# tonyzyl/ladcast

Hardware: AMD Instinct MI355X
Metric: ensemble-member-steps/sec (higher is better)
Workload: dtype f32

## Files before the change

include/ladcast_hip.h:

```cpp
#ifndef LADCAST_HIP_H
#define LADCAST_HIP_H

#ifdef __cplusplus
extern "C" {
#endif

#define LDC_ABI_VERSION 5

#define LDC_OK 0
#define LDC_ERR_ARG (-1)
#define LDC_ERR_ALIGN (-2)
#define LDC_ERR_UNSUPPORTED (-3)

enum ldc_act { LDC_ACT_NONE = 0, LDC_ACT_SILU = 1, LDC_ACT_GELU_TANH = 2, LDC_ACT_RELU = 3 };
#define LDC_ACT_IN_TIMESTEP_SINCOS 16

int ldc_abi_version(void);
const char* ldc_build_arch(void);

typedef struct ldc_gemm_desc {
  int M, N, K, batch;
  int lda, ldw, ldc, ldr;
  long long a_bs, c_bs, r_bs;
  int gate_bs;
  int act;
  int flags;
  int reserved;
} ldc_gemm_desc;
#define LDC_GEMM_A_SPLIT 1
#define LDC_GEMM_C_SPLIT 2
#define LDC_GEMM_BF16_1TERM 4
#define LDC_GEMM_F32_REGSTAGE 8
#define LDC_FMT_F32 0
#define LDC_FMT_SPLIT 1
#define LDC_FMT_BF16 2
int ldc_sizeof_gemm_desc(void);
int ldc_gemm_bias_act(const float* A, const float* W, const float* bias, const float* gate,
                      const float* R, float* C, const ldc_gemm_desc* d, void* stream);

#define LDC_GEMM_MAX_PROBLEMS 4
typedef struct ldc_gemm_problem {
  const float* A;
  const float* W;
  const float* bias;
  const float* gate;
  const float* R;
  float* C;
  ldc_gemm_desc d;
} ldc_gemm_problem;
int ldc_sizeof_gemm_problem(void);
long long ldc_gemm_grouped_workspace_bytes(void);
int ldc_gemm_grouped_workspace_init(void* workspace, long long workspace_bytes, void* stream);
int ldc_gemm_grouped(const ldc_gemm_problem* problems, int n, void* workspace, long long workspace_bytes,
// ... 66 lines not shown
int ldc_attn_fwd_split_qrows(const float* Q, const float* K, const float* V, float* O, int B, int S, int Sq, int H, int ld_qkv,
                             long long qkv_bs, int ldo, long long o_bs, const float* key_bias, int flags, void* workspace,
                             long long workspace_bytes, void* stream);

int ldc_qk_rmsnorm_rope(float* q, float* k, int B, int row0, int rows, int H, int ld, long long bs,
                        const float* wq, const float* wk, float eps, const float* cos_tab,
                        const float* sin_tab, void* stream);

int ldc_layernorm_mod(const float* x, float* y, int B, int rows, int D, int ldx, long long x_bs,
                      int ldy, long long y_bs, const float* scale, const float* shift, int mod_bs,
                      int mode, float eps, int out_split, void* stream);
int ldc_layernorm_mod2(const float* x, float* y, int B, int rows, int D, int ldx, long long x_bs,
                       int ldy, long long y_bs, const float* scale, const float* shift, int split_row,
                       const float* scale2, const float* shift2, int mod_bs, int mode, float eps,
                       int out_split, void* stream);

int ldc_mean_rows(const float* x, float* y, int B, int rows, int D, int ldx, long long x_bs, void* stream);
int ldc_mean_rows_split(const float* x, float* y, float* x_split, int B, int rows, int D, int ldx,
                        long long x_bs, int lds, long long s_bs, int fmt , void* stream);

int ldc_gate_residual(const float* resid, const float* y, const float* gate, float* out, int B,
                      int rows, int D, int ld_res, long long res_bs, int ld_y, long long y_bs,
                      int gate_bs, void* stream);
int ldc_gate_residual_layernorm(float* resid, const float* y, const float* gate, float* out, int B, int rows, int D, int ld_res,
                                long long res_bs, int ld_y, long long y_bs, int gate_bs, int ld_out, long long out_bs,
                                const float* weight, const float* bias, float eps, int out_split, void* stream);

int ldc_chan_to_token(const float* in, float* out, int B, int C, int N, int ldo, int fill_cols, void* stream);
int ldc_chan_to_token_split(const float* in, float* out, int B, int C, int N, int ldo, int fill_cols,
                            int out_split, void* stream);
// ... 202 lines not shown
```

ladcast_amd/csrc/gemm_f32.hip:

```cpp
#include "common.h"

namespace {

constexpr int BM = 128, BN = 128, BK = 32;
constexpr int LDP = 36;
constexpr int STAGE_FLOATS = (BM + BN) * LDP;

struct GemmArgs {
  const float* A;
  const float* W;
  const float* bias;
  const float* gate;
  const float* R;
  float* C;
  ldc_gemm_desc d;
  int cH, cW, cin, ks;
};

__device__ __forceinline__ int sphere_src_pixel(int h, int w, int ky, int kx, int H, int W, int ks) {
  const int p = ks >> 1;
  if ((h == 0 && ky < p) || (h == H - 1 && ky >= ks - p)) kx = ks - 1 - kx;
  int r = h + ky - p;
  int c = w + kx - p;
  if (r < 0) {
    r = -1 - r;
    c -= W >> 1;
  } else if (r >= H) {
    r = 2 * H - 1 - r;
    c -= W >> 1;
  }
  c %= W;
// ... 67 lines not shown
        rb[i] = (kin && gn < N) ? *reinterpret_cast<const float4*>(W + static_cast<long long>(gn) * ldw + kk)
                                : make_float4(0.f, 0.f, 0.f, 0.f);
      }
    }
  };
  auto sstore = [&](int stage) {
    float* As = smem + stage * STAGE_FLOATS;
    float* Bs = As + BM * LDP;
#pragma unroll
    for (int i = 0; i < 4; ++i) {
      const int row = r0 + 32 * i;
      *reinterpret_cast<float4*>(As + row * LDP + c4 * 4) = ra[i];
      *reinterpret_cast<float4*>(Bs + row * LDP + c4 * 4) = rb[i];
    }
  };

  f32x16 acc[2][2];
#pragma unroll
  for (int i = 0; i < 2; ++i)
#pragma unroll
    for (int j = 0; j < 2; ++j)
#pragma unroll
      for (int r = 0; r < 16; ++r) acc[i][j][r] = 0.f;

  const int nk = CONV ? ktpt * p.ks * p.ks : (K + BK - 1) / BK;
  gload(0);
  sstore(0);
  __syncthreads();

  const int frag_row = lane & 31;
  const int frag_k = (lane >> 5) * 4;

  for (int kt = 0; kt < nk; ++kt) {
    if (kt + 1 < nk) gload(kt + 1);
    const float* As = smem + (kt & 1) * STAGE_FLOATS;
    const float* Bs = As + BM * LDP;
    const float* a_base = As + (wm * 64 + frag_row) * LDP + frag_k;
    const float* b_base = Bs + (wn * 64 + frag_row) * LDP + frag_k;
#pragma unroll
    for (int kg = 0; kg < 4; ++kg) {
      const float4 a0 = *reinterpret_cast<const float4*>(a_base + kg * 8);
      const float4 a1 = *reinterpret_cast<const float4*>(a_base + 32 * LDP + kg * 8);
      const float4 b0 = *reinterpret_cast<const float4*>(b_base + kg * 8);
      const float4 b1 = *reinterpret_cast<const float4*>(b_base + 32 * LDP + kg * 8);
      const float av[2][4] = {{a0.x, a0.y, a0.z, a0.w}, {a1.x, a1.y, a1.z, a1.w}};
      const float bv[2][4] = {{b0.x, b0.y, b0.z, b0.w}, {b1.x, b1.y, b1.z, b1.w}};
#pragma unroll
      for (int r = 0; r < 4; ++r)
#pragma unroll
        for (int i = 0; i < 2; ++i)
#pragma unroll
          for (int j = 0; j < 2; ++j)
            acc[i][j] = __builtin_amdgcn_mfma_f32_32x32x2f32(av[i][r], bv[j][r], acc[i][j], 0, 0, 0);
    }
    if (kt + 1 < nk) sstore((kt + 1) & 1);
    __syncthreads();
  }

  float* __restrict__ C = p.C + static_cast<long long>(b) * p.d.c_bs;
  const float* __restrict__ R = p.R ? p.R + static_cast<long long>(b) * p.d.r_bs : nullptr;
  const float* __restrict__ gate = p.gate ? p.gate + static_cast<long long>(b) * p.d.gate_bs : nullptr;
  const int act = p.d.act;
#pragma unroll
  for (int j = 0; j < 2; ++j) {
    const int n = bn * BN + wn * 64 + j * 32 + (lane & 31);
    if (n >= N) continue;
    const float bias_n = p.bias ? p.bias[n] : 0.f;
    const float gate_n = gate ? gate[n] : 1.f;
#pragma unroll
    for (int i = 0; i < 2; ++i) {
#pragma unroll
// ... 15 lines not shown
extern "C" int ldc_sizeof_gemm_desc(void) { return static_cast<int>(sizeof(ldc_gemm_desc)); }

extern "C" int ldc_gemm_bias_act(const float* A, const float* W, const float* bias, const float* gate,
                                 const float* R, float* C, const ldc_gemm_desc* d, void* stream) {
  LDC_CHECK_PTR(A);
  LDC_CHECK_PTR(W);
  LDC_CHECK_PTR(C);
  LDC_CHECK_PTR(d);
  if (d->M <= 0 || d->N <= 0 || d->K <= 0 || d->batch <= 0) return LDC_ERR_ARG;
  LDC_CHECK_ALIGN16(A);
  LDC_CHECK_ALIGN16(W);
  if ((d->K & 3) || (d->lda & 3) || (d->ldw & 3) || (d->a_bs & 3)) return LDC_ERR_ALIGN;
  if (d->act < LDC_ACT_NONE || d->act > LDC_ACT_RELU) return LDC_ERR_UNSUPPORTED;
  if (d->flags != 0) return LDC_ERR_UNSUPPORTED;
  if (d->batch > 65535 || ldc_cdiv(d->M, BM) > 65535) return LDC_ERR_UNSUPPORTED;
  GemmArgs p{A, W, bias, gate, R, C, *d, 0, 0, 0, 0};
  dim3 grid(ldc_cdiv(d->N, BN), ldc_cdiv(d->M, BM), d->batch);
  const size_t lds = 2 * STAGE_FLOATS * sizeof(float);
  static const bool attr_set = [&] {
    (void)hipFuncSetAttribute(reinterpret_cast<const void*>(gemm_nt_f32_kernel<false>),
                              hipFuncAttributeMaxDynamicSharedMemorySize, static_cast<int>(lds));
    return true;
  }();
  (void)attr_set;
  hipLaunchKernelGGL(gemm_nt_f32_kernel<false>, grid, dim3(256), lds, static_cast<hipStream_t>(stream), p);
  return ldc_launch_status();
}

extern "C" int ldc_sphere_conv_nhwc(const float* X, const float* Wt, const float* bias, const float* R, float* Y,
                                    int B, int H, int W, int cin, int ldx, int cout, int ldy, int ldr, int ksize,
                                    int act, void* stream) {
// ... 7 lines not shown
  LDC_CHECK_ALIGN16(Wt);
  if ((cin & 3) || (ldx & 3) || ldx < cin || ldy < cout) return LDC_ERR_ALIGN;
  if (act < LDC_ACT_NONE || act > LDC_ACT_RELU) return LDC_ERR_UNSUPPORTED;
  const long long M = static_cast<long long>(B) * H * W;
  if (M > 0x7fffffffLL || ldc_cdiv(M, BM) > 65535) return LDC_ERR_UNSUPPORTED;
  ldc_gemm_desc d{};
  d.M = static_cast<int>(M);
  d.N = cout;
  d.K = ksize * ksize * cin;
  d.batch = 1;
  d.lda = ldx;
  d.ldw = ksize * ksize * cin;
  d.ldc = ldy;
  d.ldr = ldr;
  d.act = act;
  GemmArgs p{X, Wt, bias, nullptr, R, Y, d, H, W, cin, ksize};
  dim3 grid(ldc_cdiv(cout, BN), ldc_cdiv(M, BM), 1);
  const size_t lds = 2 * STAGE_FLOATS * sizeof(float);
  static const bool attr_set = [&] {
    (void)hipFuncSetAttribute(reinterpret_cast<const void*>(gemm_nt_f32_kernel<true>),
                              hipFuncAttributeMaxDynamicSharedMemorySize, static_cast<int>(lds));
    return true;
  }();
  (void)attr_set;
  hipLaunchKernelGGL(gemm_nt_f32_kernel<true>, grid, dim3(256), lds, static_cast<hipStream_t>(stream), p);
  return ldc_launch_status();
}
```

ladcast_amd/csrc/rowops.hip:

```cpp
#include "common.h"

namespace {

constexpr int LN_MAX_V4 = 8;

__global__ __launch_bounds__(256) void layernorm_mod_kernel(float* __restrict__ x, float* __restrict__ y,
                                                            int rows, int D, int ldx, long long x_bs, int ldy,
                                                            long long y_bs, const float* __restrict__ scale,
                                                            const float* __restrict__ shift, int split_row,
                                                            const float* __restrict__ scale2,
                                                            const float* __restrict__ shift2, int mod_bs, int mode,
                                                            float eps, int out_split, const float* __restrict__ pre_y,
                                                            const float* __restrict__ pre_gate, int ld_prey,
                                                            long long prey_bs, int gate_bs) {
  const int lane = threadIdx.x & 63;
  const int row = blockIdx.x * 4 + (threadIdx.x >> 6);
  const int b = blockIdx.y;
  if (row >= rows) return;
  if (row >= split_row) {
    scale = scale2;
    shift = shift2;
  }
  float* xr = x + b * x_bs + static_cast<long long>(row) * ldx;
  float* yr = y + b * y_bs + static_cast<long long>(row) * ldy;
  const int nv4 = D >> 2;
  float4 v[LN_MAX_V4];
  float sum = 0.f;
#pragma unroll
  for (int i = 0; i < LN_MAX_V4; ++i) {
    const int c = lane + 64 * i;
    if (c < nv4) {
      v[i] = reinterpret_cast<const float4*>(xr)[c];
      if (pre_y) {
        const float4 yv = reinterpret_cast<const float4*>(pre_y + b * prey_bs + static_cast<long long>(row) * ld_prey)[c];
        const float4 g = reinterpret_cast<const float4*>(pre_gate + static_cast<long long>(b) * gate_bs)[c];
        v[i] = make_float4(fmaf(yv.x, g.x, v[i].x), fmaf(yv.y, g.y, v[i].y), fmaf(yv.z, g.z, v[i].z), fmaf(yv.w, g.w, v[i].w));
        reinterpret_cast<float4*>(xr)[c] = v[i];
      }
// ... 385 lines not shown
}

struct LSGroup {
  ldc_linear_small_problem p[LDC_LINEAR_SMALL_MAX_GROUPED];
};

__global__ __launch_bounds__(256) void linear_small_grouped_kernel(LSGroup g) {
  const ldc_linear_small_problem& q = g.p[blockIdx.z];
  if (static_cast<int>(blockIdx.x) * 4 >= q.N || static_cast<int>(blockIdx.y) * LS_ROWS >= q.rows) return;
  const int kc = q.K < LS_KC ? q.K : LS_KC;
  linear_small_body<1>(q.x, q.x_rows, q.W, q.bias, q.add, q.add_rows, q.y, q.rows, q.N, q.K, kc, q.act_in, q.act_out, 1);
}

}

extern "C" int ldc_layernorm_mod2(const float* x, float* y, int B, int rows, int D, int ldx, long long x_bs, int ldy,
                                  long long y_bs, const float* scale, const float* shift, int split_row,
                                  const float* scale2, const float* shift2, int mod_bs, int mode, float eps,
                                  int out_split, void* stream) {
  LDC_CHECK_PTR(x);
  LDC_CHECK_PTR(y);
  if (B <= 0 || rows <= 0 || D <= 0 || split_row < 0) return LDC_ERR_ARG;
  if ((D & 3) || D > 64 * 4 * LN_MAX_V4) return LDC_ERR_UNSUPPORTED;
  if ((ldx & 3) || (ldy & 3) || (x_bs & 3) || (y_bs & 3) || (mod_bs & 3)) return LDC_ERR_ALIGN;
  LDC_CHECK_ALIGN16(x);
  LDC_CHECK_ALIGN16(y);
  if (scale) LDC_CHECK_ALIGN16(scale);
  if (shift) LDC_CHECK_ALIGN16(shift);
  if (scale2) LDC_CHECK_ALIGN16(scale2);
  if (shift2) LDC_CHECK_ALIGN16(shift2);
  if (mode != 0 && mode != 1) return LDC_ERR_UNSUPPORTED;
  if (out_split && ((D & 7) || (ldy & 7) || (y_bs & 7) || (reinterpret_cast<unsigned long long>(y) & 31ull))) return LDC_ERR_ALIGN;
  dim3 grid(ldc_cdiv(rows, 4), B);
  hipLaunchKernelGGL(layernorm_mod_kernel, grid, dim3(256), 0, static_cast<hipStream_t>(stream), const_cast<float*>(x), y, rows, D,
                     ldx, x_bs, ldy, y_bs, scale, shift, split_row, scale2, shift2, mod_bs, mode, eps, out_split,
                     static_cast<const float*>(nullptr), static_cast<const float*>(nullptr), 0, 0LL, 0);
  return ldc_launch_status();
}

extern "C" int ldc_gate_residual_layernorm(float* resid, const float* yv, const float* gate, float* out, int B, int rows, int D,
                                           int ld_res, long long res_bs, int ld_y, long long y_bs, int gate_bs, int ld_out,
                                           long long out_bs, const float* weight, const float* bias, float eps, int out_split,
                                           void* stream) {
  LDC_CHECK_PTR(resid);
  LDC_CHECK_PTR(yv);
  LDC_CHECK_PTR(gate);
  LDC_CHECK_PTR(out);
  if (B <= 0 || rows <= 0 || D <= 0) return LDC_ERR_ARG;
  if ((D & 3) || D > 64 * 4 * LN_MAX_V4) return LDC_ERR_UNSUPPORTED;
  if ((ld_res & 3) || (ld_y & 3) || (ld_out & 3) || (res_bs & 3) || (y_bs & 3) || (out_bs & 3) || (gate_bs & 3)) return LDC_ERR_ALIGN;
  LDC_CHECK_ALIGN16(resid);
  LDC_CHECK_ALIGN16(yv);
  LDC_CHECK_ALIGN16(gate);
  LDC_CHECK_ALIGN16(out);
  if (weight) LDC_CHECK_ALIGN16(weight);
  if (bias) LDC_CHECK_ALIGN16(bias);
  if (out_split && ((D & 7) || (ld_out & 7) || (out_bs & 7) || (reinterpret_cast<unsigned long long>(out) & 31ull))) return LDC_ERR_ALIGN;
  dim3 grid(ldc_cdiv(rows, 4), B);
  hipLaunchKernelGGL(layernorm_mod_kernel, grid, dim3(256), 0, static_cast<hipStream_t>(stream), resid, out, rows, D, ld_res, res_bs,
                     ld_out, out_bs, weight, bias, rows, static_cast<const float*>(nullptr), static_cast<const float*>(nullptr), 0, 1,
                     eps, out_split, yv, gate, ld_y, y_bs, gate_bs);
  return ldc_launch_status();
}

extern "C" int ldc_layernorm_mod(const float* x, float* y, int B, int rows, int D, int ldx, long long x_bs, int ldy,
                                 long long y_bs, const float* scale, const float* shift, int mod_bs, int mode,
                                 float eps, int out_split, void* stream) {
  return ldc_layernorm_mod2(x, y, B, rows, D, ldx, x_bs, ldy, y_bs, scale, shift, rows, nullptr, nullptr, mod_bs, mode, eps,
                            out_split, stream);
}

extern "C" int ldc_qk_rmsnorm_rope(float* q, float* k, int B, int row0, int rows, int H, int ld, long long bs,
                                   const float* wq, const float* wk, float eps, const float* cos_tab,
                                   const float* sin_tab, void* stream) {
  LDC_CHECK_PTR(q);
  LDC_CHECK_PTR(k);
// ... 198 lines not shown
```

ladcast_amd/hip.py:

```python
from __future__ import annotations

import ctypes
import os
from ctypes import POINTER, Structure, c_char_p, c_double, c_float, c_int, c_longlong, c_void_p

import torch

_HERE = os.path.dirname(os.path.abspath(__file__))
LIB_PATH = os.environ.get("LDC_LIB_PATH") or os.path.join(_HERE, "libladcast_hip.so")

ACT_NONE, ACT_SILU, ACT_GELU_TANH, ACT_RELU = 0, 1, 2, 3
ACT_IN_TIMESTEP_SINCOS = 16
GEMM_A_SPLIT, GEMM_C_SPLIT, GEMM_BF16_1TERM = 1, 2, 4
GEMM_F32_REGSTAGE = 8
ATTN_OUT_SPLIT, ATTN_BF16_1TERM, ATTN_OUT_BF16 = 1, 2, 4
ABI_VERSION = 5
FMT_F32, FMT_SPLIT, FMT_BF16 = 0, 1, 2


class GemmDesc(Structure):
    _fields_ = [
        ("M", c_int), ("N", c_int), ("K", c_int), ("batch", c_int),
        ("lda", c_int), ("ldw", c_int), ("ldc", c_int), ("ldr", c_int),
        ("a_bs", c_longlong), ("c_bs", c_longlong), ("r_bs", c_longlong),
# ... 47 lines not shown


def _load():
    if not os.path.exists(LIB_PATH):
        raise RuntimeError(
            f"{LIB_PATH} is missing: build it with `python -c 'import __graft_entry__ as g; g.build()'` "
            "(or `make -C ladcast_amd/csrc`).  ladcast_amd has no CPU fallback."
        )
    lib = ctypes.CDLL(LIB_PATH)
    P, I, L, F, D = c_void_p, c_int, c_longlong, c_float, c_double
    sig = {
        "ldc_abi_version": (I, []),
        "ldc_build_arch": (c_char_p, []),
        "ldc_sizeof_gemm_desc": (I, []),
        "ldc_gemm_bias_act": (I, [P, P, P, P, P, P, POINTER(GemmDesc), P]),
        "ldc_sizeof_gemm_problem": (I, []),
        "ldc_gemm_grouped_workspace_bytes": (L, []),
        "ldc_gemm_grouped_workspace_init": (I, [P, L, P]),
        "ldc_gemm_grouped": (I, [POINTER(GemmProblem), I, P, L, P]),
        "ldc_gemm_grouped_bf16x3": (I, [POINTER(GemmProblem), I, P, L, P]),
        "ldc_sizeof_qkv_epilogue": (I, []),
        "ldc_gemm_grouped_bf16x3_qkv": (I, [POINTER(GemmProblem), POINTER(QkvEpilogue), I, P, L, P]),
        "ldc_gemm_grouped_qkv_f32": (I, [POINTER(GemmProblem), POINTER(QkvEpilogue), I, P, L, P]),
        "ldc_attn_qkv_prepare_split": (I, [P, P, P, I, I, I, I, L, I, P, P, P, P, P, P, P, P, F, P]),
        "ldc_attn_fwd_split_workspace_bytes": (L, [I, I, I]),
        "ldc_attn_fwd_split_workspace_max_bytes": (L, []),
        "ldc_attn_fwd_split": (I, [P, P, P, P, I, I, I, I, L, I, L, P, I, P, L, P]),
        "ldc_attn_fwd_split_qrows_workspace_bytes": (L, [I, I, I, I]),
        "ldc_attn_fwd_split_qrows": (I, [P, P, P, P, I, I, I, I, I, L, I, L, P, I, P, L, P]),
        "ldc_pack_weight_bf16x2": (I, [P, P, I, I, I, P]),
# ... 30 lines not shown
        "ldc_rollout_spectrum_workspace_bytes": (L, [I, I, I, I, I]),
        "ldc_rollout_spectrum": (I, [P, L, L, L, P, P, F, P, L, L, P, P, I, I, I, I, I, P, P, I, I, P, L, P]),
        "ldc_sizeof_products_desc": (I, []),
        "ldc_rollout_products": (I, [P, L, L, L, P, P, F, P, I, I, I, I, I, I, POINTER(ProductsDesc), P, P, P, P, I, I, P]),
        "ldc_sizeof_events_desc": (I, []),
        "ldc_rollout_events_workspace_bytes": (L, [I, I, I, I, I]),
        "ldc_rollout_events": (I, [P, L, L, L, P, P, F, P, L, L, P, P, L, L, P, P, I, I, I, I, I, POINTER(EventsDesc), P, P, P, I, I, P, L, P]),
        "ldc_rollout_fss_workspace_bytes": (L, [I, I, I, I, I, I]),
        "ldc_rollout_fss": (I, [P, L, L, L, P, P, F, P, L, L, P, P, L, L, P, P, I, I, I, I, I, POINTER(EventsDesc), POINTER(c_int), I, P, P, I, I, P, L, P]),
        "ldc_rollout_regional_workspace_bytes": (L, [I, I, I, I, I, I]),
        "ldc_rollout_regional": (I, [P, L, L, L, P, P, F, P, L, L, P, P, L, L, P, P, P, I, I, I, I, I, I, P, P, I, I, P, L, P]),
        "ldc_rollout_energy_workspace_bytes": (L, [I, I, I, I, I, I]),
        "ldc_rollout_energy": (I, [P, L, L, L, P, P, F, P, L, L, P, P, P, P, I, I, I, I, I, I, P, P, P, P, I, I, P, L, P]),
        "ldc_layernorm_mod": (I, [P, P, I, I, I, I, L, I, L, P, P, I, I, F, I, P]),
        "ldc_layernorm_mod2": (I, [P, P, I, I, I, I, L, I, L, P, P, I, P, P, I, I, F, I, P]),
        "ldc_mean_rows": (I, [P, P, I, I, I, I, L, P]),
        "ldc_mean_rows_split": (I, [P, P, P, I, I, I, I, L, I, L, I, P]),
        "ldc_chan_to_token_split": (I, [P, P, I, I, I, I, I, I, P]),
        "ldc_gate_residual": (I, [P, P, P, P, I, I, I, I, L, I, L, I, P]),
        "ldc_chan_to_token": (I, [P, P, I, I, I, I, I, P]),
        "ldc_token_to_chan": (I, [P, P, I, I, I, I, P]),
        "ldc_timestep_embedding": (I, [P, P, I, P]),
        "ldc_temb_modulate": (I, [P, P, I, I, I, P]),
        "ldc_chan_affine": (I, [P, P, P, P, F, L, I, L, I, P]),
        "ldc_edm_scale_f64_to_f32": (I, [P, D, P, L, P]),
        "ldc_edm_init_state": (I, [P, D, P, L, P]),
        "ldc_edm_euler": (I, [P, P, D, D, D, D, P, P, L, P]),
        "ldc_edm_churn": (I, [P, P, c_double, P, L, P]),
        "ldc_edm_heun": (I, [P, P, P, P, D, D, D, D, L, P]),
        "ldc_f64_to_f32": (I, [P, P, L, P]),
# ... 70 lines not shown

def _dev(*ts):
    for t in ts:
        if t is not None and not t.is_cuda:
            raise RuntimeError("ladcast_amd kernels need device tensors (no CPU fallback)")


def gemm(A, W, C, *, M, N, K, batch=1, lda=None, ldw=None, ldc=None, a_bs=0, c_bs=0, bias=None, gate=None,
         gate_bs=0, R=None, ldr=0, r_bs=0, act=ACT_NONE):
    _dev(A, W, C, bias, gate, R)
    d = GemmDesc(M, N, K, batch, lda if lda is not None else K, ldw if ldw is not None else K,
                 ldc if ldc is not None else N, ldr, a_bs, c_bs, r_bs, gate_bs, act, 0, 0)
    _check(lib.ldc_gemm_bias_act(_p(A), _p(W), _p(bias), _p(gate), _p(R), _p(C), ctypes.byref(d), _stream()), "ldc_gemm_bias_act")


_workspaces = {}
_outgrown = []


def _workspace(name, device, nbytes, init=None, grow=False):
    key = (name, str(device), torch.cuda.current_stream(device).cuda_stream)
    ws = _workspaces.get(key)
    if ws is None or (grow and ws.numel() * 4 < nbytes):
        if not grow and torch.cuda.is_current_stream_capturing():
            raise RuntimeError(f"{name}: the first call on a stream must be made outside a graph capture (run one warm-up forward)")
        if ws is not None:
            _outgrown.append(ws)
        ws = torch.empty((nbytes + 3) // 4, device=device, dtype=torch.float32)
        if init == "zero":
            ws.zero_()
# ... 408 lines not shown

def pad_key_bias(bias):
    S = bias.numel()
    out = torch.zeros(32 * ((S + 31) // 32), device=bias.device, dtype=torch.float32)
    out[:S] = bias.reshape(-1)
    return out


def qk_rmsnorm_rope(q, k, *, B, row0, rows, H, ld, bs, wq, wk, eps, cos=None, sin=None):
    _dev(q, k, wq, wk, cos, sin)
    _check(lib.ldc_qk_rmsnorm_rope(_p(q), _p(k), B, row0, rows, H, ld, bs, _p(wq), _p(wk), eps, _p(cos), _p(sin), _stream()),
           "ldc_qk_rmsnorm_rope")


def layernorm_mod(x, y, *, B, rows, D, ldx, x_bs, ldy, y_bs, scale=None, shift=None, mod_bs=0, mode=0, eps=1e-6, out_split=False,
                  split_row=None, scale2=None, shift2=None):
    _dev(x, y, scale, shift, scale2, shift2)
    if split_row is None:
        _check(lib.ldc_layernorm_mod(_p(x), _p(y), B, rows, D, ldx, x_bs, ldy, y_bs, _p(scale), _p(shift), mod_bs, mode, eps,
                                     int(out_split), _stream()),
               "ldc_layernorm_mod")
    else:
        _check(lib.ldc_layernorm_mod2(_p(x), _p(y), B, rows, D, ldx, x_bs, ldy, y_bs, _p(scale), _p(shift), split_row, _p(scale2), _p(shift2),
                                      mod_bs, mode, eps, int(out_split), _stream()),
               "ldc_layernorm_mod2")


def mean_rows(x, y, *, B, rows, D, ldx, x_bs, x_split=None, lds=None, s_bs=None, fmt=FMT_SPLIT):
    _dev(x, y, x_split)
    if x_split is None:
        _check(lib.ldc_mean_rows(_p(x), _p(y), B, rows, D, ldx, x_bs, _stream()), "ldc_mean_rows")
    else:
        _check(lib.ldc_mean_rows_split(_p(x), _p(y), _p(x_split), B, rows, D, ldx, x_bs, lds if lds is not None else ldx,
# ... 303 lines not shown
```

ladcast_amd/models/LaDCast_3D_model.py:

```python
from __future__ import annotations

from types import SimpleNamespace
from typing import Optional, Tuple

import numpy as np
import torch
import torch.nn as nn

from .. import graphs, hip
from .embeddings import get_year_sincos_embedding, rope_tables_from_grid, rotary_1d
from .modeling_utils import ModelMixin


class _RMSNormP(nn.Module):
    def __init__(self, dim, eps):
        super().__init__()
        self.eps = eps
        self.weight = nn.Parameter(torch.ones(dim))

    def forward(self, x):
        var = x.to(torch.float32).pow(2).mean(-1, keepdim=True)
        return x * torch.rsqrt(var + self.eps) * self.weight


# ... 532 lines not shown
        if Bt not in (1, B):
            raise ValueError(f"timestep must have 1 or {B} entries, got {Bt}")
        te = None
        if time_elapsed is not None and self.time_elapsed_embed is not None:
            te = self._time_elapsed_embedding(time_elapsed, dev)
            if te.shape[0] not in (1, B):
                raise ValueError("time_elapsed must have 1 or batch entries")

        if conditioning is not None:
            pack, idx = conditioning
            if tuple(pack.shape) != (B,) + tuple(conditioning_tensors.shape[1:]) or not 0 <= idx < pack.levels:
                raise ValueError("`conditioning` was prepared for another batch / conditioning shape")
            out = self._main_device(hidden_states, pack, idx)
            return (out,) if not return_dict else SimpleNamespace(sample=out)
        if self.use_hip_graph:
            gkey = (B, Bt, C_in, R, T_in, Hh, Ww, None if te is None else (te.data_ptr(), te.shape[0]), bool(self.skip_unread_rows))
            inputs = [hidden_states, timestep, conditioning_tensors]
            ent = self._graphs.get(gkey)
            if ent is None:
                ent = self._graphs[gkey] = graphs.capture(lambda x, t, k: self._forward_device(x, t, k, te), inputs, dev, self.capture_stream())
            out = ent.replay(*inputs)
        else:
            out = self._forward_device(hidden_states, timestep, conditioning_tensors, te)
        if not return_dict:
            return (out,)
        return SimpleNamespace(sample=out)

    def time_elapsed_embedding(self, time_elapsed):
        if time_elapsed is None or self.time_elapsed_embed is None:
            return None
        if self._plan is None:
# ... 10 lines not shown
            self._capture_stream = torch.cuda.Stream(device=self.device)
        return self._capture_stream

    @torch.no_grad()
    def forward_launch_only(self, hidden_states, timestep, conditioning_tensors, te, conditioning=None):
        if self._plan is None:
            self._build_plan()
        if hidden_states.dtype != torch.float32 or not hidden_states.is_cuda or not hidden_states.is_contiguous():
            raise TypeError("forward_launch_only takes a contiguous fp32 device tensor (use forward() for anything else)")
        if conditioning is not None:
            return self._main_device(hidden_states, conditioning[0], conditioning[1])
        return self._forward_device(hidden_states, timestep.reshape(-1), conditioning_tensors, te)

    batch_conditioning = True
    skip_unread_rows = True
    COND_MAX_ROWS = 96

    @torch.no_grad()
    def prepare_conditioning(self, timesteps, conditioning_tensors, te=None):
        if self._plan is None:
            self._build_plan()
        dev = self.device
        timesteps = timesteps.to(device=dev, dtype=torch.float32).reshape(-1)
        conditioning_tensors = conditioning_tensors.to(device=dev, dtype=torch.float32)
        if conditioning_tensors.dim() != 5:
            raise ValueError("conditioning_tensors must be (B, C, T_in, h, w)")
        N, B = timesteps.shape[0], conditioning_tensors.shape[0]
        shape = tuple(conditioning_tensors.shape)
        per = max(1, self.COND_MAX_ROWS // B)
        if per >= N:
# ... 141 lines not shown
        C_out = (cfg.out_channels or cfg.in_channels) * self._patch_vol
        kpad = max(plan.kx_pad, plan.kc_pad)
        key = (B, Nx, Nc, kpad)
        if key not in self._ws:
            self._ws[key] = _Workspace(dev, B, 1, Nx, Nc, D, kpad, C_out, 4)
        ws = self._ws[key]
        pc, ps, cc, cs, pk, ck, jk = self._rope_tables(R, T_in, Hh, Ww, dev)
        SD = S * D
        h_x, h_c = ws.h[:, :Nx], ws.h[:, Nx:]
        nh_x, nh_c = ws.nh[:, :Nx], ws.nh[:, Nx:]
        NM = plan.mod_w.shape[0]
        mods = pack.mods[idx * B : (idx + 1) * B]
        split = plan.split

        AS, CS, fmt, G, run, run1, run_qkv = self._launchers(plan)

        if split:
            KX = plan.kx_pad
            xtok = ws.xtok.view(-1)[: B * Nx * KX].view(B, Nx, KX)
            hip.chan_to_token(hidden_states, xtok, B=B, C=C_in, N=Nx, ldo=KX, fill_cols=KX, out_split=fmt)
            run1(xtok, plan.wx, h_x, M=Nx, N=D, K=KX, batch=B, a_bs=Nx * KX, c_bs=SD, bias=self.x_embedder.proj.bias, flags=AS)
        else:
            hip.chan_to_token(hidden_states, ws.xtok.view(-1)[: B * Nx * C_in].view(B, Nx, C_in), B=B, C=C_in, N=Nx, ldo=C_in)
            hip.gemm(ws.xtok, plan.wx, h_x, M=Nx, N=D, K=C_in, batch=B, a_bs=Nx * C_in, c_bs=SD, bias=self.x_embedder.proj.bias)
        h_c.copy_(pack.ctx[idx * B : (idx + 1) * B])

        kb_all = None
        if self.scale_attn_by_lat:
            if Hh * Ww != self.attn_lat_weights.numel():
                raise ValueError("scale_attn_by_lat is hard-wired to the 15 x 30 latent grid (models/LaDCast_3D_model.py:684-692)")
            kb_all = self._key_bias(R + T_in, dev)
        foreign = bool(self._foreign_processors())
        m_all = None
        if foreign:
            if split:
                raise NotImplementedError("a user-supplied attention processor runs on the fp32 path: call set_gemm_precision('fp32') "
                                          "(or change the attention arithmetic through the C ABI, include/ladcast_hip.h)")
            if torch.cuda.is_current_stream_capturing():
                raise NotImplementedError("a user-supplied attention processor cannot be captured into a hipGraph")
            if self.scale_attn_by_lat:
                w = self.attn_lat_weights.to(dev)
                m_all = w.repeat(1, 1, 1, T_in + R)


        def mod_of(linear, width):
            o = plan.mod_off[id(linear)]
            return mods[:, o : o + width]

        for blk in self.transformer_blocks:
            pa = plan.attn[id(blk.attn)]
            mx, mc = mod_of(blk.norm1.linear, 6 * D), mod_of(blk.norm1_context.linear, 6 * D)
            hip.layernorm_mod(ws.h, ws.nh, B=B, rows=S, D=D, ldx=D, x_bs=SD, ldy=D, y_bs=SD, scale=mx[:, D:], shift=mx, split_row=Nx, scale2=mc[:, D:], shift2=mc,
                              mod_bs=NM, mode=0, eps=1e-6, out_split=fmt)
            if blk.attn.foreign_processor is not None:
                a, ca = self._call_processor(blk.attn, nh_x, nh_c, m_all, (pc, ps), (cc, cs))
                a, ca = a.contiguous(), ca.contiguous()
                hip.gate_residual(h_x, a, mx[:, 2 * D :], h_x, B=B, rows=Nx, D=D, ld_res=D, res_bs=SD, ld_y=D, y_bs=Nx * D, gate_bs=NM)
                hip.gate_residual(h_c, ca, mc[:, 2 * D :], h_c, B=B, rows=Nc, D=D, ld_res=D, res_bs=SD, ld_y=D, y_bs=Nc * D, gate_bs=NM)
            else:
                nd = run_qkv([
                    G(nh_x, pa.wqkv, ws.qkv, M=Nx, N=3 * D, K=D, batch=B, a_bs=SD, c_bs=S * 3 * D, bias=pa.bqkv, flags=AS),
                    G(nh_c, pa.wqkv_c, ws.qkv[:, Nx:], M=Nc, N=3 * D, K=D, batch=B, a_bs=SD, c_bs=S * 3 * D, bias=pa.bqkv_c, flags=AS),
                ], [self._qkv_epi(blk.attn.norm_q, blk.attn.norm_k, pk), self._qkv_epi(blk.attn.norm_added_q, blk.attn.norm_added_k, None)])
                self._attention(ws, B, 0, Nx, Nc, ws.att, D, SD, (blk.attn.norm_q, blk.attn.norm_k, pc, ps),
                                (blk.attn.norm_added_q, blk.attn.norm_added_k, None, None), out_split=fmt, key_bias=kb_all, normed=nd)
                o, oc = blk.attn.to_out[0], blk.attn.to_add_out
                run([
                    G(ws.att, o.weight, h_x, M=Nx, N=D, K=D, batch=B, a_bs=SD, c_bs=SD, bias=o.bias, gate=mx[:, 2 * D :], gate_bs=NM, R=h_x, ldr=D, r_bs=SD, flags=AS),
                    G(ws.att[:, Nx:], oc.weight, h_c, M=Nc, N=D, K=D, batch=B, a_bs=SD, c_bs=SD, bias=oc.bias, gate=mc[:, 2 * D :], gate_bs=NM, R=h_c, ldr=D, r_bs=SD, flags=AS),
                ])
            hip.layernorm_mod(ws.h, ws.nh, B=B, rows=S, D=D, ldx=D, x_bs=SD, ldy=D, y_bs=SD, scale=mx[:, 4 * D :], shift=mx[:, 3 * D :], split_row=Nx,
                              scale2=mc[:, 4 * D :], shift2=mc[:, 3 * D :], mod_bs=NM, mode=0, eps=1e-7, out_split=fmt)
            up, down = [], []
            for (hs, nhs, rows, ff, mod, off) in ((h_x, nh_x, Nx, blk.ff, mx, 0), (h_c, nh_c, Nc, blk.ff_context, mc, Nx)):
                f0, f2 = ff.net[0].proj, ff.net[2]
                F = f0.weight.shape[0]
                hid = ws.cat.view(-1)[off * B * F :]
                up.append(G(nhs, f0.weight, hid, M=rows, N=F, K=D, batch=B, a_bs=SD, c_bs=rows * F, bias=f0.bias, act=hip.ACT_GELU_TANH, flags=AS | CS))
                down.append(G(hid, f2.weight, hs, M=rows, N=D, K=F, batch=B, a_bs=rows * F, c_bs=SD, bias=f2.bias,
                              gate=mod[:, 5 * D :], gate_bs=NM, R=hs, ldr=D, r_bs=SD, flags=AS))
            run(up)
            run(down)

        n_single = len(self.single_transformer_blocks)
# ... 32 lines not shown
```

ladcast_amd/pipelines/edm_sampler.py:

```python
from __future__ import annotations

from typing import List, Optional, Union

import numpy as np
import torch

from .. import graphs, hip
from .torch_utils import randn_tensor


@torch.no_grad()
def edm_AR_sampler(
    net,
    noise_scheduler,
    batch_size=1,
    return_seq_len=1,
    randn_like=torch.randn_like,
    num_inference_steps=18,
    S_churn=0,
    S_min=0,
    S_max=float("inf"),
    S_noise=0,
    deterministic=True,
    known_latents=None,
# ... 21 lines not shown
    known = known.contiguous()

    chunk_graph = bool(getattr(net, "use_hip_graph", False)) and hasattr(net, "forward_launch_only") and hasattr(net, "_graphs")
    batched = bool(getattr(net, "batch_conditioning", False)) and hasattr(net, "prepare_conditioning")
    if not deterministic:
        out = torch.empty(shape, device=device, dtype=torch.float32)
        fwd = lambda x, t, k, te_: net(x, t, k, time_elapsed=timestamps).sample
        _heun_chunk_stochastic(fwd, noise_scheduler, t_steps, latents, known, out, shape, device, num_inference_steps, randn_like, S_churn, S_min,
                               S_max, S_noise)
        return out
    if chunk_graph:
        te = net.time_elapsed_embedding(timestamps)
        plan_id = net.plan_identity()
        key = (tuple(shape), tuple(known.shape), num_inference_steps, tuple(float(v) for v in t_steps.tolist()),
               None if te is None else (te.data_ptr(), tuple(te.shape)), str(device), plan_id, batched,
               bool(getattr(net, "skip_unread_rows", False)))
        prepare = net.prepare_conditioning if batched else None
        key = ("edm_chunk",) + key
        cache = net._graphs
        turn = cache.get(key + ("turn",), 0)
        cache[key + ("turn",)] = turn ^ 1

        def capture():
            st_out, cn = torch.empty(shape, device=device, dtype=torch.float32), c_noise_host.to(device)

            def chunk(lat, kn):
                _heun_chunk(net.forward_launch_only, noise_scheduler, t_steps, cn, lat, kn, te, st_out, shape, device, num_inference_steps, prepare)
                return st_out

            return graphs.capture(chunk, [latents, known], device, net.capture_stream(), keep=cn)

# ... 68 lines not shown
```

ladcast_amd/pipelines/pipeline_AR.py:

```python
from __future__ import annotations

from typing import List, Optional, Tuple, Union

import torch

from .. import graphs
from .torch_utils import randn_tensor
from .utils import Fields2DPipelineOutput


class AutoRegressive2DPipeline:
    model_cpu_offload_seq = "unet"

    def __init__(self, ar_model, scheduler, scheduler_step_kwargs: Optional[dict] = None):
        self.register_modules(ar_model=ar_model, scheduler=scheduler)
        self.scheduler_step_kwargs = scheduler_step_kwargs or {}

    def register_modules(self, **mods):
        for k, v in mods.items():
            setattr(self, k, v)

    @property
    def _execution_device(self):
        return self.ar_model.device
# ... 53 lines not shown
            t_host = t
            t = t.expand(batch_size).to(dev)
            t.host_value = t_host
            ckw = {} if pack is None else {"conditioning": (pack, i)}
            model_output = self.ar_model(x_in, t, known_latents, time_elapsed=timestamps, return_dict=False, **ckw)[0]
            image = self.scheduler.step(model_output, t, image, **self.scheduler_step_kwargs, return_dict=False)[0]
        if not return_dict:
            return (image,)
        return Fields2DPipelineOutput(fields=image)

    def _graph_loop(self, net, sch, image, known, timestamps, num_inference_steps, batch_size, dev):
        sch.set_timesteps(num_inference_steps)
        te = net.time_elapsed_embedding(timestamps)
        key = (tuple(image.shape), tuple(known.shape), num_inference_steps, sch.graph_signature(),
               tuple(sorted((k, str(v)) for k, v in self.scheduler_step_kwargs.items())), None if te is None else (te.data_ptr(), tuple(te.shape)), str(dev), net.plan_identity(),
               bool(getattr(net, "batch_conditioning", False)), bool(getattr(net, "skip_unread_rows", False)))
        key = ("pipeline_loop",) + key
        cache = net._graphs
        ent = cache.get(key)
        if ent is None:
            ts_dev = sch.timesteps.to(device=dev, dtype=torch.float32).contiguous()
            tsteps = [t.to(device=dev, dtype=torch.float32).expand(batch_size).contiguous() for t in sch.timesteps]

            def loop(img, kn):
                kb = kn if kn.shape[0] == batch_size else kn.expand(batch_size, *kn.shape[1:]).contiguous()
                pack = net.prepare_conditioning(ts_dev, kb, te) if getattr(net, "batch_conditioning", False) else None
                for i, (t, t_dev) in enumerate(zip(sch.timesteps, tsteps)):
                    x_in = sch.scale_model_input(img, t)
                    out = net.forward_launch_only(x_in, t_dev, kb, te, None if pack is None else (pack, i))
                    img = sch.step(out, t, img, **self.scheduler_step_kwargs, return_dict=False)[0]
                return img
# ... 9 lines not shown
```

Before: 3.244.

## Fuse input transpose into GEMM and read context rows in place

Adds a k-major A-operand path to the f32 MFMA GEMM, so the patch embedding reads channel-major hidden states directly instead of running a separate chan_to_token transpose. It also lets the first block's layernorm and residual GEMM read the conditioning context straight from the pack, which removes the h_c copy. The aim is fewer kernel launches and less memory traffic at the start of the forward pass. The cost is strided scalar LDS stores in the new A-load path and more branching in the GEMM kernel.

Result: no change. 3.246, median of 2 (+0.1%).

```diff
diff --git a/include/ladcast_hip.h b/include/ladcast_hip.h
--- a/include/ladcast_hip.h
+++ b/include/ladcast_hip.h
@@ -37,6 +37,8 @@
 int ldc_sizeof_gemm_desc(void);
 int ldc_gemm_bias_act(const float* A, const float* W, const float* bias, const float* gate,
                       const float* R, float* C, const ldc_gemm_desc* d, void* stream);
+int ldc_gemm_bias_act_kmajor(const float* A, const float* W, const float* bias, const float* gate,
+                             const float* R, float* C, const ldc_gemm_desc* d, void* stream);
 
 #define LDC_GEMM_MAX_PROBLEMS 4
 typedef struct ldc_gemm_problem {
@@ -133,6 +135,10 @@
                        int ldy, long long y_bs, const float* scale, const float* shift, int split_row,
                        const float* scale2, const float* shift2, int mod_bs, int mode, float eps,
                        int out_split, void* stream);
+int ldc_layernorm_mod2_src2(const float* x, const float* x2, int ldx2, long long x2_bs, float* y, int B, int rows, int D,
+                            int ldx, long long x_bs, int ldy, long long y_bs, const float* scale, const float* shift,
+                            int split_row, const float* scale2, const float* shift2, int mod_bs, int mode, float eps,
+                            int out_split, void* stream);
 
 int ldc_mean_rows(const float* x, float* y, int B, int rows, int D, int ldx, long long x_bs, void* stream);
 int ldc_mean_rows_split(const float* x, float* y, float* x_split, int B, int rows, int D, int ldx,
diff --git a/ladcast_amd/csrc/gemm_f32.hip b/ladcast_amd/csrc/gemm_f32.hip
--- a/ladcast_amd/csrc/gemm_f32.hip
+++ b/ladcast_amd/csrc/gemm_f32.hip
@@ -15,6 +15,7 @@
   float* C;
   ldc_gemm_desc d;
   int cH, cW, cin, ks;
+  int a_kmajor;
 };
 
 __device__ __forceinline__ int sphere_src_pixel(int h, int w, int ky, int kx, int H, int W, int ks) {
@@ -112,6 +113,37 @@
       *reinterpret_cast<float4*>(Bs + row * LDP + c4 * 4) = rb[i];
     }
   };
+  auto gload_at = [&](int kt, float4 (&qa)[4]) {
+#pragma unroll
+    for (int i = 0; i < 4; ++i) {
+      const int kk = kt * BK + c4 + 8 * i;
+      const int gm = bm * BM + 4 * r0;
+      qa[i] = (kk < K && gm < M) ? *reinterpret_cast<const float4*>(A + static_cast<long long>(kk) * lda + gm)
+                                 : make_float4(0.f, 0.f, 0.f, 0.f);
+    }
+  };
+  auto gload_w = [&](int kt, float4 (&qb)[4]) {
+    const int kk = kt * BK + c4 * 4;
+#pragma unroll
+    for (int i = 0; i < 4; ++i) {
+      const int gn = bn * BN + r0 + 32 * i;
+      qb[i] = (kk < K && gn < N) ? *reinterpret_cast<const float4*>(W + static_cast<long long>(gn) * ldw + kk)
+                                 : make_float4(0.f, 0.f, 0.f, 0.f);
+    }
+  };
+  auto sstore_at = [&](int stage, const float4 (&qa)[4], const float4 (&qb)[4]) {
+    float* As = smem + stage * STAGE_FLOATS;
+    float* Bs = As + BM * LDP;
+#pragma unroll
+    for (int i = 0; i < 4; ++i) {
+      float* a = As + 4 * r0 * LDP + c4 + 8 * i;
+      a[0] = qa[i].x;
+      a[LDP] = qa[i].y;
+      a[2 * LDP] = qa[i].z;
+      a[3 * LDP] = qa[i].w;
+      *reinterpret_cast<float4*>(Bs + (r0 + 32 * i) * LDP + c4 * 4) = qb[i];
+    }
+  };
 
   f32x16 acc[2][2];
 #pragma unroll
@@ -122,16 +154,10 @@
       for (int r = 0; r < 16; ++r) acc[i][j][r] = 0.f;
 
   const int nk = CONV ? ktpt * p.ks * p.ks : (K + BK - 1) / BK;
-  gload(0);
-  sstore(0);
-  __syncthreads();
-
   const int frag_row = lane & 31;
   const int frag_k = (lane >> 5) * 4;
-
-  for (int kt = 0; kt < nk; ++kt) {
-    if (kt + 1 < nk) gload(kt + 1);
-    const float* As = smem + (kt & 1) * STAGE_FLOATS;
+  auto mma = [&](int stage) {
+    const float* As = smem + stage * STAGE_FLOATS;
     const float* Bs = As + BM * LDP;
     const float* a_base = As + (wm * 64 + frag_row) * LDP + frag_k;
     const float* b_base = Bs + (wn * 64 + frag_row) * LDP + frag_k;
@@ -151,8 +177,63 @@
           for (int j = 0; j < 2; ++j)
             acc[i][j] = __builtin_amdgcn_mfma_f32_32x32x2f32(av[i][r], bv[j][r], acc[i][j], 0, 0, 0);
     }
-    if (kt + 1 < nk) sstore((kt + 1) & 1);
+  };
+
+  bool done = false;
+  if constexpr (!CONV) {
+    if (p.a_kmajor) {
+      done = true;
+      if (nk <= 3) {
+        float4 qa[3][4], qb[3][4];
+#pragma unroll
+        for (int t = 0; t < 3; ++t)
+          if (t < nk) {
+            gload_at(t, qa[t]);
+            gload_w(t, qb[t]);
+          }
+        sstore_at(0, qa[0], qb[0]);
+        if (nk > 1) sstore_at(1, qa[1], qb[1]);
+        __syncthreads();
+        mma(0);
+        if (nk > 1) {
+          if (nk > 2) {
+            __syncthreads();
+            sstore_at(0, qa[2], qb[2]);
+          }
+          mma(1);
+          if (nk > 2) {
+            __syncthreads();
+            mma(0);
+          }
+        }
+      } else {
+        float4 qa[4], qb[4];
+        gload_at(0, qa);
+        gload_w(0, qb);
+        sstore_at(0, qa, qb);
+        __syncthreads();
+        for (int kt = 0; kt < nk; ++kt) {
+          if (kt + 1 < nk) {
+            gload_at(kt + 1, qa);
+            gload_w(kt + 1, qb);
+          }
+          mma(kt & 1);
+          if (kt + 1 < nk) sstore_at((kt + 1) & 1, qa, qb);
+          __syncthreads();
+        }
+      }
+    }
+  }
+  if (!done) {
+    gload(0);
+    sstore(0);
     __syncthreads();
+    for (int kt = 0; kt < nk; ++kt) {
+      if (kt + 1 < nk) gload(kt + 1);
+      mma(kt & 1);
+      if (kt + 1 < nk) sstore((kt + 1) & 1);
+      __syncthreads();
+    }
   }
 
   float* __restrict__ C = p.C + static_cast<long long>(b) * p.d.c_bs;
@@ -198,7 +279,34 @@
   if (d->act < LDC_ACT_NONE || d->act > LDC_ACT_RELU) return LDC_ERR_UNSUPPORTED;
   if (d->flags != 0) return LDC_ERR_UNSUPPORTED;
   if (d->batch > 65535 || ldc_cdiv(d->M, BM) > 65535) return LDC_ERR_UNSUPPORTED;
-  GemmArgs p{A, W, bias, gate, R, C, *d, 0, 0, 0, 0};
+  GemmArgs p{A, W, bias, gate, R, C, *d, 0, 0, 0, 0, 0};
+  dim3 grid(ldc_cdiv(d->N, BN), ldc_cdiv(d->M, BM), d->batch);
+  const size_t lds = 2 * STAGE_FLOATS * sizeof(float);
+  static const bool attr_set = [&] {
+    (void)hipFuncSetAttribute(reinterpret_cast<const void*>(gemm_nt_f32_kernel<false>),
+                              hipFuncAttributeMaxDynamicSharedMemorySize, static_cast<int>(lds));
+    return true;
+  }();
+  (void)attr_set;
+  hipLaunchKernelGGL(gemm_nt_f32_kernel<false>, grid, dim3(256), lds, static_cast<hipStream_t>(stream), p);
+  return ldc_launch_status();
+}
+
+extern "C" int ldc_gemm_bias_act_kmajor(const float* A, const float* W, const float* bias, const float* gate, const float* R,
+                                        float* C, const ldc_gemm_desc* d, void* stream) {
+  LDC_CHECK_PTR(A);
+  LDC_CHECK_PTR(W);
+  LDC_CHECK_PTR(C);
+  LDC_CHECK_PTR(d);
+  if (d->M <= 0 || d->N <= 0 || d->K <= 0 || d->batch <= 0) return LDC_ERR_ARG;
+  if (d->lda < d->M) return LDC_ERR_ARG;
+  LDC_CHECK_ALIGN16(A);
+  LDC_CHECK_ALIGN16(W);
+  if ((d->M & 3) || (d->K & 3) || (d->lda & 3) || (d->ldw & 3) || (d->a_bs & 3)) return LDC_ERR_ALIGN;
+  if (d->act < LDC_ACT_NONE || d->act > LDC_ACT_RELU) return LDC_ERR_UNSUPPORTED;
+  if (d->flags != 0) return LDC_ERR_UNSUPPORTED;
+  if (d->batch > 65535 || ldc_cdiv(d->M, BM) > 65535) return LDC_ERR_UNSUPPORTED;
+  GemmArgs p{A, W, bias, gate, R, C, *d, 0, 0, 0, 0, 1};
   dim3 grid(ldc_cdiv(d->N, BN), ldc_cdiv(d->M, BM), d->batch);
   const size_t lds = 2 * STAGE_FLOATS * sizeof(float);
   static const bool attr_set = [&] {
@@ -236,7 +344,7 @@
   d.ldc = ldy;
   d.ldr = ldr;
   d.act = act;
-  GemmArgs p{X, Wt, bias, nullptr, R, Y, d, H, W, cin, ksize};
+  GemmArgs p{X, Wt, bias, nullptr, R, Y, d, H, W, cin, ksize, 0};
   dim3 grid(ldc_cdiv(cout, BN), ldc_cdiv(M, BM), 1);
   const size_t lds = 2 * STAGE_FLOATS * sizeof(float);
   static const bool attr_set = [&] {
diff --git a/ladcast_amd/csrc/rowops.hip b/ladcast_amd/csrc/rowops.hip
--- a/ladcast_amd/csrc/rowops.hip
+++ b/ladcast_amd/csrc/rowops.hip
@@ -12,16 +12,18 @@
                                                             const float* __restrict__ shift2, int mod_bs, int mode,
                                                             float eps, int out_split, const float* __restrict__ pre_y,
                                                             const float* __restrict__ pre_gate, int ld_prey,
-                                                            long long prey_bs, int gate_bs) {
+                                                            long long prey_bs, int gate_bs, const float* __restrict__ x2,
+                                                            int ldx2, long long x2_bs) {
   const int lane = threadIdx.x & 63;
   const int row = blockIdx.x * 4 + (threadIdx.x >> 6);
   const int b = blockIdx.y;
   if (row >= rows) return;
+  float* xr = x + b * x_bs + static_cast<long long>(row) * ldx;
   if (row >= split_row) {
     scale = scale2;
     shift = shift2;
-  }
-  float* xr = x + b * x_bs + static_cast<long long>(row) * ldx;
+    if (x2) xr = const_cast<float*>(x2) + b * x2_bs + static_cast<long long>(row - split_row) * ldx2;
+  }
   float* yr = y + b * y_bs + static_cast<long long>(row) * ldy;
   const int nv4 = D >> 2;
   float4 v[LN_MAX_V4];
@@ -437,12 +439,16 @@
 
 }
 
-extern "C" int ldc_layernorm_mod2(const float* x, float* y, int B, int rows, int D, int ldx, long long x_bs, int ldy,
-                                  long long y_bs, const float* scale, const float* shift, int split_row,
-                                  const float* scale2, const float* shift2, int mod_bs, int mode, float eps,
-                                  int out_split, void* stream) {
+static int layernorm_mod2_impl(const float* x, const float* x2, int ldx2, long long x2_bs, float* y, int B, int rows, int D, int ldx,
+                               long long x_bs, int ldy, long long y_bs, const float* scale, const float* shift, int split_row,
+                               const float* scale2, const float* shift2, int mod_bs, int mode, float eps, int out_split,
+                               void* stream) {
   LDC_CHECK_PTR(x);
   LDC_CHECK_PTR(y);
+  if (x2) {
+    if ((ldx2 & 3) || (x2_bs & 3)) return LDC_ERR_ALIGN;
+    LDC_CHECK_ALIGN16(x2);
+  }
   if (B <= 0 || rows <= 0 || D <= 0 || split_row < 0) return LDC_ERR_ARG;
   if ((D & 3) || D > 64 * 4 * LN_MAX_V4) return LDC_ERR_UNSUPPORTED;
   if ((ldx & 3) || (ldy & 3) || (x_bs & 3) || (y_bs & 3) || (mod_bs & 3)) return LDC_ERR_ALIGN;
@@ -457,8 +463,25 @@
   dim3 grid(ldc_cdiv(rows, 4), B);
   hipLaunchKernelGGL(layernorm_mod_kernel, grid, dim3(256), 0, static_cast<hipStream_t>(stream), const_cast<float*>(x), y, rows, D,
                      ldx, x_bs, ldy, y_bs, scale, shift, split_row, scale2, shift2, mod_bs, mode, eps, out_split,
-                     static_cast<const float*>(nullptr), static_cast<const float*>(nullptr), 0, 0LL, 0);
+                     static_cast<const float*>(nullptr), static_cast<const float*>(nullptr), 0, 0LL, 0, x2, ldx2, x2_bs);
   return ldc_launch_status();
+}
+
+extern "C" int ldc_layernorm_mod2(const float* x, float* y, int B, int rows, int D, int ldx, long long x_bs, int ldy,
+                                  long long y_bs, const float* scale, const float* shift, int split_row,
+                                  const float* scale2, const float* shift2, int mod_bs, int mode, float eps,
+                                  int out_split, void* stream) {
+  return layernorm_mod2_impl(x, nullptr, 0, 0, y, B, rows, D, ldx, x_bs, ldy, y_bs, scale, shift, split_row, scale2, shift2, mod_bs, mode,
+                             eps, out_split, stream);
+}
+
+extern "C" int ldc_layernorm_mod2_src2(const float* x, const float* x2, int ldx2, long long x2_bs, float* y, int B, int rows, int D,
+                                       int ldx, long long x_bs, int ldy, long long y_bs, const float* scale, const float* shift,
+                                       int split_row, const float* scale2, const float* shift2, int mod_bs, int mode, float eps,
+                                       int out_split, void* stream) {
+  LDC_CHECK_PTR(x2);
+  return layernorm_mod2_impl(x, x2, ldx2, x2_bs, y, B, rows, D, ldx, x_bs, ldy, y_bs, scale, shift, split_row, scale2, shift2, mod_bs,
+                             mode, eps, out_split, stream);
 }
 
 extern "C" int ldc_gate_residual_layernorm(float* resid, const float* yv, const float* gate, float* out, int B, int rows, int D,
@@ -482,7 +505,7 @@
   dim3 grid(ldc_cdiv(rows, 4), B);
   hipLaunchKernelGGL(layernorm_mod_kernel, grid, dim3(256), 0, static_cast<hipStream_t>(stream), resid, out, rows, D, ld_res, res_bs,
                      ld_out, out_bs, weight, bias, rows, static_cast<const float*>(nullptr), static_cast<const float*>(nullptr), 0, 1,
-                     eps, out_split, yv, gate, ld_y, y_bs, gate_bs);
+                     eps, out_split, yv, gate, ld_y, y_bs, gate_bs, static_cast<const float*>(nullptr), 0, 0LL);
   return ldc_launch_status();
 }
 
diff --git a/ladcast_amd/hip.py b/ladcast_amd/hip.py
--- a/ladcast_amd/hip.py
+++ b/ladcast_amd/hip.py
@@ -85,6 +85,7 @@
         "ldc_build_arch": (c_char_p, []),
         "ldc_sizeof_gemm_desc": (I, []),
         "ldc_gemm_bias_act": (I, [P, P, P, P, P, P, POINTER(GemmDesc), P]),
+        "ldc_gemm_bias_act_kmajor": (I, [P, P, P, P, P, P, POINTER(GemmDesc), P]),
         "ldc_sizeof_gemm_problem": (I, []),
         "ldc_gemm_grouped_workspace_bytes": (L, []),
         "ldc_gemm_grouped_workspace_init": (I, [P, L, P]),
@@ -145,6 +146,7 @@
         "ldc_rollout_energy": (I, [P, L, L, L, P, P, F, P, L, L, P, P, P, P, I, I, I, I, I, I, P, P, P, P, I, I, P, L, P]),
         "ldc_layernorm_mod": (I, [P, P, I, I, I, I, L, I, L, P, P, I, I, F, I, P]),
         "ldc_layernorm_mod2": (I, [P, P, I, I, I, I, L, I, L, P, P, I, P, P, I, I, F, I, P]),
+        "ldc_layernorm_mod2_src2": (I, [P, P, I, L, P, I, I, I, I, L, I, L, P, P, I, P, P, I, I, F, I, P]),
         "ldc_mean_rows": (I, [P, P, I, I, I, I, L, P]),
         "ldc_mean_rows_split": (I, [P, P, P, I, I, I, I, L, I, L, I, P]),
         "ldc_chan_to_token_split": (I, [P, P, I, I, I, I, I, I, P]),
@@ -245,6 +247,20 @@
     _check(lib.ldc_gemm_bias_act(_p(A), _p(W), _p(bias), _p(gate), _p(R), _p(C), ctypes.byref(d), _stream()), "ldc_gemm_bias_act")
 
 
+ERR_ALIGN = -2
+
+
+def gemm_kmajor(A, W, C, *, M, N, K, lda, batch=1, ldw=None, ldc=None, a_bs=0, c_bs=0, bias=None, gate=None, gate_bs=0, R=None, ldr=0, r_bs=0,
+                act=ACT_NONE):
+    _dev(A, W, C, bias, gate, R)
+    d = GemmDesc(M, N, K, batch, lda, ldw if ldw is not None else K, ldc if ldc is not None else N, ldr, a_bs, c_bs, r_bs, gate_bs, act, 0, 0)
+    st = lib.ldc_gemm_bias_act_kmajor(_p(A), _p(W), _p(bias), _p(gate), _p(R), _p(C), ctypes.byref(d), _stream())
+    if st == ERR_ALIGN:
+        return False
+    _check(st, "ldc_gemm_bias_act_kmajor")
+    return True
+
+
 _workspaces = {}
 _outgrown = []
 
@@ -683,9 +699,13 @@
 
 
 def layernorm_mod(x, y, *, B, rows, D, ldx, x_bs, ldy, y_bs, scale=None, shift=None, mod_bs=0, mode=0, eps=1e-6, out_split=False,
-                  split_row=None, scale2=None, shift2=None):
-    _dev(x, y, scale, shift, scale2, shift2)
-    if split_row is None:
+                  split_row=None, scale2=None, shift2=None, x2=None, ldx2=None, x2_bs=0):
+    _dev(x, y, scale, shift, scale2, shift2, x2)
+    if x2 is not None:
+        _check(lib.ldc_layernorm_mod2_src2(_p(x), _p(x2), ldx2 if ldx2 is not None else ldx, x2_bs, _p(y), B, rows, D, ldx, x_bs, ldy, y_bs,
+                                           _p(scale), _p(shift), split_row, _p(scale2), _p(shift2), mod_bs, mode, eps, int(out_split),
+                                           _stream()), "ldc_layernorm_mod2_src2")
+    elif split_row is None:
         _check(lib.ldc_layernorm_mod(_p(x), _p(y), B, rows, D, ldx, x_bs, ldy, y_bs, _p(scale), _p(shift), mod_bs, mode, eps,
                                      int(out_split), _stream()),
                "ldc_layernorm_mod")
diff --git a/ladcast_amd/models/LaDCast_3D_model.py b/ladcast_amd/models/LaDCast_3D_model.py
--- a/ladcast_amd/models/LaDCast_3D_model.py
+++ b/ladcast_amd/models/LaDCast_3D_model.py
@@ -570,7 +570,8 @@
             out = self._main_device(hidden_states, pack, idx)
             return (out,) if not return_dict else SimpleNamespace(sample=out)
         if self.use_hip_graph:
-            gkey = (B, Bt, C_in, R, T_in, Hh, Ww, None if te is None else (te.data_ptr(), te.shape[0]), bool(self.skip_unread_rows))
+            gkey = (B, Bt, C_in, R, T_in, Hh, Ww, None if te is None else (te.data_ptr(), te.shape[0]), bool(self.skip_unread_rows),
+                    bool(self.fused_forward_ends))
             inputs = [hidden_states, timestep, conditioning_tensors]
             ent = self._graphs.get(gkey)
             if ent is None:
@@ -611,6 +612,7 @@
 
     batch_conditioning = True
     skip_unread_rows = True
+    fused_forward_ends = True
     COND_MAX_ROWS = 96
 
     @torch.no_grad()
@@ -782,6 +784,7 @@
         split = plan.split
 
         AS, CS, fmt, G, run, run1, run_qkv = self._launchers(plan)
+        fused = bool(self.fused_forward_ends) and not split
 
         if split:
             KX = plan.kx_pad
@@ -789,9 +792,15 @@
             hip.chan_to_token(hidden_states, xtok, B=B, C=C_in, N=Nx, ldo=KX, fill_cols=KX, out_split=fmt)
             run1(xtok, plan.wx, h_x, M=Nx, N=D, K=KX, batch=B, a_bs=Nx * KX, c_bs=SD, bias=self.x_embedder.proj.bias, flags=AS)
         else:
-            hip.chan_to_token(hidden_states, ws.xtok.view(-1)[: B * Nx * C_in].view(B, Nx, C_in), B=B, C=C_in, N=Nx, ldo=C_in)
-            hip.gemm(ws.xtok, plan.wx, h_x, M=Nx, N=D, K=C_in, batch=B, a_bs=Nx * C_in, c_bs=SD, bias=self.x_embedder.proj.bias)
-        h_c.copy_(pack.ctx[idx * B : (idx + 1) * B])
+            if not (fused and hip.gemm_kmajor(hidden_states, plan.wx, h_x, M=Nx, N=D, K=C_in, lda=Nx, batch=B, a_bs=C_in * Nx, c_bs=SD,
+                                              bias=self.x_embedder.proj.bias)):
+                hip.chan_to_token(hidden_states, ws.xtok.view(-1)[: B * Nx * C_in].view(B, Nx, C_in), B=B, C=C_in, N=Nx, ldo=C_in)
+                hip.gemm(ws.xtok, plan.wx, h_x, M=Nx, N=D, K=C_in, batch=B, a_bs=Nx * C_in, c_bs=SD, bias=self.x_embedder.proj.bias)
+        ctx = pack.ctx[idx * B : (idx + 1) * B]
+        ctx_in_place = (fused and len(self.transformer_blocks) > 0 and self.transformer_blocks[0].attn.foreign_processor is None
+                        and tuple(ctx.shape) == (B, Nc, D) and ctx.is_contiguous())
+        if not ctx_in_place:
+            h_c.copy_(ctx)
 
         kb_all = None
         if self.scale_attn_by_lat:
@@ -815,11 +824,12 @@
             o = plan.mod_off[id(linear)]
             return mods[:, o : o + width]
 
-        for blk in self.transformer_blocks:
+        for i_blk, blk in enumerate(self.transformer_blocks):
             pa = plan.attn[id(blk.attn)]
             mx, mc = mod_of(blk.norm1.linear, 6 * D), mod_of(blk.norm1_context.linear, 6 * D)
+            in_place = ctx_in_place and i_blk == 0
             hip.layernorm_mod(ws.h, ws.nh, B=B, rows=S, D=D, ldx=D, x_bs=SD, ldy=D, y_bs=SD, scale=mx[:, D:], shift=mx, split_row=Nx, scale2=mc[:, D:], shift2=mc,
-                              mod_bs=NM, mode=0, eps=1e-6, out_split=fmt)
+                              mod_bs=NM, mode=0, eps=1e-6, out_split=fmt, x2=ctx if in_place else None, ldx2=D, x2_bs=Nc * D)
             if blk.attn.foreign_processor is not None:
                 a, ca = self._call_processor(blk.attn, nh_x, nh_c, m_all, (pc, ps), (cc, cs))
                 a, ca = a.contiguous(), ca.contiguous()
@@ -835,7 +845,8 @@
                 o, oc = blk.attn.to_out[0], blk.attn.to_add_out
                 run([
                     G(ws.att, o.weight, h_x, M=Nx, N=D, K=D, batch=B, a_bs=SD, c_bs=SD, bias=o.bias, gate=mx[:, 2 * D :], gate_bs=NM, R=h_x, ldr=D, r_bs=SD, flags=AS),
-                    G(ws.att[:, Nx:], oc.weight, h_c, M=Nc, N=D, K=D, batch=B, a_bs=SD, c_bs=SD, bias=oc.bias, gate=mc[:, 2 * D :], gate_bs=NM, R=h_c, ldr=D, r_bs=SD, flags=AS),
+                    G(ws.att[:, Nx:], oc.weight, h_c, M=Nc, N=D, K=D, batch=B, a_bs=SD, c_bs=SD, bias=oc.bias, gate=mc[:, 2 * D :], gate_bs=NM, R=ctx if in_place else h_c, ldr=D,
+                      r_bs=Nc * D if in_place else SD, flags=AS),
                 ])
             hip.layernorm_mod(ws.h, ws.nh, B=B, rows=S, D=D, ldx=D, x_bs=SD, ldy=D, y_bs=SD, scale=mx[:, 4 * D :], shift=mx[:, 3 * D :], split_row=Nx,
                               scale2=mc[:, 4 * D :], shift2=mc[:, 3 * D :], mod_bs=NM, mode=0, eps=1e-7, out_split=fmt)
diff --git a/ladcast_amd/pipelines/edm_sampler.py b/ladcast_amd/pipelines/edm_sampler.py
--- a/ladcast_amd/pipelines/edm_sampler.py
+++ b/ladcast_amd/pipelines/edm_sampler.py
@@ -59,7 +59,8 @@
         plan_id = net.plan_identity()
         key = (tuple(shape), tuple(known.shape), num_inference_steps, tuple(float(v) for v in t_steps.tolist()),
                None if te is None else (te.data_ptr(), tuple(te.shape)), str(device), plan_id, batched,
-               bool(getattr(net, "skip_unread_rows", False)))
+               bool(getattr(net, "skip_unread_rows", False)),
+               bool(getattr(net, "fused_forward_ends", False)))
         prepare = net.prepare_conditioning if batched else None
         key = ("edm_chunk",) + key
         cache = net._graphs
diff --git a/ladcast_amd/pipelines/pipeline_AR.py b/ladcast_amd/pipelines/pipeline_AR.py
--- a/ladcast_amd/pipelines/pipeline_AR.py
+++ b/ladcast_amd/pipelines/pipeline_AR.py
@@ -91,7 +91,8 @@
         te = net.time_elapsed_embedding(timestamps)
         key = (tuple(image.shape), tuple(known.shape), num_inference_steps, sch.graph_signature(),
                tuple(sorted((k, str(v)) for k, v in self.scheduler_step_kwargs.items())), None if te is None else (te.data_ptr(), tuple(te.shape)), str(dev), net.plan_identity(),
-               bool(getattr(net, "batch_conditioning", False)), bool(getattr(net, "skip_unread_rows", False)))
+               bool(getattr(net, "batch_conditioning", False)), bool(getattr(net, "skip_unread_rows", False)),
+               bool(getattr(net, "fused_forward_ends", False)))
         key = ("pipeline_loop",) + key
         cache = net._graphs
         ent = cache.get(key)
```
